# KLab/YAIK

Hardware: NVIDIA B200
Metric: encoded megapixels/sec (gradient+range stages) (higher is better)
Workload: dtype int32

## Files before the change

yaik_b200/csrc/yk_emit.cu:

```cuda
#include "yk_device.h"
#ifdef YK_EMULATE
#include <assert.h>
#endif

#ifndef YK_OWNER_THREADS
#define YK_OWNER_THREADS 256
#endif
static __device__ __forceinline__ int yk_owner_point(const YkSlotDev& S, int idx, const YkRun& run) {
    uint32_t word = __ldg(&S.touchMap[idx]);
    const int gy = idx / S.latW, gx = idx - gy * S.latW;
    if (S.hasAbove && gy == 0) word |= __ldg(&S.touchInTop[gx]);
    if (S.hasBelow && gy == S.latH - 1) word |= __ldg(&S.touchInBottom[gx]);
    if (word == 0u || (word & 0x80000000u)) return -1;
    const int rp = (__ffs((int)(word & 0x0FFFFFFFu)) - 1) >> 2;
    const unsigned nib = (word >> (4 * rp)) & 15u;
    const int pid = run.passId[rp];
    const YkGeomS g = yk_geom_s(pid);
    const int nSwzX = (S.w + (1 << g.lbw) - 1) >> g.lbw;
    const int LX = (4 * gx) >> g.shx, LY = (4 * gy) >> g.shy;
    const int tileRows = S.h >> g.shy;
    int best = INT_MAX, bestK = 0;
#pragma unroll
    for (int k = 0; k < 4; k++) {
        if ((nib >> k) & 1u) {
            const int ty = LY - (k >> 1);
            int pos;
            if (ty < 0) pos = k - 5;
            else if (ty >= tileRows) pos = INT_MAX - 1;
            else pos = yk_pos_s(g, nSwzX, LX - (k & 1), ty);
            if (pos < best) { best = pos; bestK = k; }
        }
    }
    if (best < 0 || best == INT_MAX - 1) return -1;
    atomicOr(&S.emitNib[pid][best >> 3], 1u << (4 * (best & 7) + bestK));
    return (pid << 24) | (int)((unsigned)(best >> 3) / YK_EMIT_THREADS);
}

static __device__ __forceinline__ void yk_rgb_add(const YkSlotDev& S, int key, unsigned bytes) {
    const unsigned grp = (unsigned)key & 0xFFFFFFu;
    atomicAdd(&S.rgbTot[key >> 24][grp], bytes);
    atomicAdd(&S.rgbSup[key >> 24][grp / YK_SUPER], bytes);
}
static __device__ __forceinline__ void yk_r2_add(const YkSlotDev& S, int grp, unsigned sum) {
    const unsigned long long v = (unsigned long long)(sum >> 16) << 32 | (sum & 0xFFFFu);
    atomicAdd(&S.r2Tot[grp], v);
    atomicAdd(&S.r2Sup[grp / YK_SUPER], v);
}

static __device__ __forceinline__ unsigned yk_r2_count(const YkSlotDev& S, int tx, int ty) {
    const uint32_t r0 = S.cellMask[(size_t)(2 * ty) * S.nbx + (tx >> 3)], r1 = S.cellMask[(size_t)(2 * ty + 1) * S.nbx + (tx >> 3)];
    const int s2 = 2 * (tx & 7);
    const unsigned chunks = 4u - (unsigned)__popc(((r0 >> s2) & 3u) | (((r1 >> s2) & 3u) << 2));
    return chunks ? chunks << 16 | 1u : 0u;
}

__global__ void __launch_bounds__(YK_OWNER_THREADS)
yk_k_owner(const YkSlotDev* __restrict__ slots, int slot0, int nPoints, int owners, YkRun run) {
    __shared__ int sKey[YK_NPASS + 1];
    __shared__ unsigned sSum[YK_NPASS + 1];
    if (threadIdx.x <= YK_NPASS) { sKey[threadIdx.x] = -1; sSum[threadIdx.x] = 0u; }
    __syncthreads();
    const YkSlotDev& S = slots[slot0 + blockIdx.y];
    const int idx = blockIdx.x * blockDim.x + threadIdx.x;
    const int lane = threadIdx.x & 31;
    const int key = owners && idx < nPoints ? yk_owner_point(S, idx, run) : -1;
    int r2Key = -1;
    unsigned r2 = 0u;
    if (run.doR2 && idx < nPoints) {
        const int gy = idx / S.latW, gx = idx - gy * S.latW, tx = gx >> 1, ty = gy >> 1;
        if (!((gx | gy) & 1) && tx < (S.w >> 3) && ty < (S.h >> 3)) {
            r2 = yk_r2_count(S, tx, ty);
            if (r2) r2Key = (int)((unsigned)(ty * (S.w >> 3) + tx) / YK_EMIT_THREADS);
        }
    }
    const unsigned rgbLanes = __ballot_sync(YK_FULL, key >= 0), r2Lanes = __ballot_sync(YK_FULL, r2Key >= 0);
    const int rgbTop = __reduce_max_sync(YK_FULL, key), r2Top = __reduce_max_sync(YK_FULL, r2Key);
    const bool rgbOne = __all_sync(YK_FULL, key < 0 || key == rgbTop), r2One = __all_sync(YK_FULL, r2Key < 0 || r2Key == r2Top);
    const unsigned r2Warp = __reduce_add_sync(YK_FULL, r2);
    const bool addRgb = key >= 0 && (!rgbOne || lane == __ffs((int)rgbLanes) - 1);
    const bool addR2 = r2Key >= 0 && (!r2One || lane == __ffs((int)r2Lanes) - 1);
    const unsigned rgbBytes = rgbOne ? 3u * (unsigned)__popc(rgbLanes) : 3u, r2Sum = r2One ? r2Warp : r2;
    if (addRgb) atomicMax(&sKey[key >> 24], key);
    if (addR2) atomicMax(&sKey[YK_NPASS], r2Key);
    __syncthreads();
    if (addRgb) {
        if (sKey[key >> 24] == key) atomicAdd(&sSum[key >> 24], rgbBytes);
        else yk_rgb_add(S, key, rgbBytes);
    }
    if (addR2) {
        if (sKey[YK_NPASS] == r2Key) atomicAdd(&sSum[YK_NPASS], r2Sum);
        else yk_r2_add(S, r2Key, r2Sum);
    }
    __syncthreads();
    if (threadIdx.x < YK_NPASS && sSum[threadIdx.x]) yk_rgb_add(S, sKey[threadIdx.x], sSum[threadIdx.x]);
    if (threadIdx.x == YK_NPASS && sSum[YK_NPASS]) yk_r2_add(S, sKey[YK_NPASS], sSum[YK_NPASS]);
}

static __device__ __forceinline__ void yk_emit_scan(unsigned c, unsigned d, unsigned pc, unsigned pd, unsigned& offC, unsigned& offD,
                                                    unsigned& totC, unsigned& totD) {
    constexpr int NW = YK_EMIT_THREADS / 32;
    __shared__ unsigned sC[NW], sD[NW], sPC[NW], sPD[NW], sTot[2];
    const int lane = threadIdx.x & 31, warp = threadIdx.x >> 5;
    unsigned ic = c, id = d;
#pragma unroll
    for (int k = 1; k < 32; k <<= 1) {
        const unsigned a0 = __shfl_up_sync(YK_FULL, ic, k), a1 = __shfl_up_sync(YK_FULL, id, k);
        if (lane >= k) { ic += a0; id += a1; }
    }
    pc = __reduce_add_sync(YK_FULL, pc); pd = __reduce_add_sync(YK_FULL, pd);
    if (lane == 31) { sC[warp] = ic; sD[warp] = id; }
    if (lane == 0) { sPC[warp] = pc; sPD[warp] = pd; }
    __syncthreads();
    if (warp == 0) {
        const unsigned a = lane < NW ? sC[lane] : 0u, b = lane < NW ? sD[lane] : 0u;
        const unsigned bc = __reduce_add_sync(YK_FULL, lane < NW ? sPC[lane] : 0u), bd = __reduce_add_sync(YK_FULL, lane < NW ? sPD[lane] : 0u);
        unsigned ia = a, ib = b;
#pragma unroll
        for (int k = 1; k < 32; k <<= 1) {
            const unsigned a0 = __shfl_up_sync(YK_FULL, ia, k), a1 = __shfl_up_sync(YK_FULL, ib, k);
            if (lane >= k) { ia += a0; ib += a1; }
        }
        if (lane < NW) { sC[lane] = bc + ia - a; sD[lane] = bd + ib - b; }
        if (lane == 31) { sTot[0] = ia; sTot[1] = ib; }
    }
    __syncthreads();
    offC = sC[warp] + ic - c; offD = sD[warp] + id - d;
    totC = sTot[0]; totD = sTot[1];
}

__global__ void __launch_bounds__(YK_EMIT_THREADS)
yk_k_emit(const YkSlotDev* __restrict__ slots, int slot0, YkRun run, int gradGroups, int r2Groups) {
    const YkSlotDev& S = slots[slot0 + blockIdx.y];
    const int tid = threadIdx.x;
    const int w = S.w, h = S.h;

    if ((int)blockIdx.x >= gradGroups) {
        const int grp = blockIdx.x - gradGroups, tilesW = w >> 3, nTiles = tilesW * (h >> 3);
        unsigned long long pre = tid < grp % YK_SUPER ? S.r2Tot[grp - grp % YK_SUPER + tid] : 0ull;
        for (int s = tid; s < grp / YK_SUPER; s += YK_EMIT_THREADS) pre += S.r2Sup[s];
        const int t = grp * YK_EMIT_THREADS + tid;
        const unsigned c = t < nTiles ? yk_r2_count(S, t % tilesW, t / tilesW) : 0u;
        const unsigned chunks = c >> 16;
        const unsigned tiles = chunks > 0;
        unsigned chunkOff, tileOff, totC, totT;
        yk_emit_scan(chunks, tiles, (unsigned)(pre >> 32), (unsigned)pre, chunkOff, tileOff, totC, totT);
#ifdef YK_EMULATE
        if (tid == 0) assert(((unsigned long long)totC << 32 | totT) == S.r2Tot[grp]);
#endif
        if (grp == r2Groups - 1 && tid == 0) { S.hdr[YK_HD_R2_CHUNKS] = (int)(chunkOff + totC); S.hdr[YK_HD_R2_TILES] = (int)(tileOff + totT); }
        if (chunks) {
#pragma unroll 1
            for (int p = 0; p < 3; p++) {
                const uint4* src = reinterpret_cast<const uint4*>(S.r2Raw[p] + (size_t)t * 64);
                uint4* dst = reinterpret_cast<uint4*>(S.r2Idx[p] + (size_t)chunkOff * 16);
                for (int k = 0; k < (int)chunks; k++) dst[k] = src[k];
                const uint32_t ty = S.r2RawType[p][t];
                uint8_t* td = S.r2Type[p] + (size_t)tileOff * 3;
                td[0] = (uint8_t)ty; td[1] = (uint8_t)(ty >> 8); td[2] = (uint8_t)(ty >> 16);
            }
        }
        return;
    }

    int rp = 0, grp = blockIdx.x, nWords = 0, nSwzX = 0, nGroups = 0;
    YkGeomS g = yk_geom_s(run.passId[0]);
    for (;;) {
        g = yk_geom_s(run.passId[rp]);
        nSwzX = (w + (1 << g.lbw) - 1) >> g.lbw;
        nWords = (nSwzX * ((h + (1 << g.lbh) - 1) >> g.lbh) * g.bits) >> 3;
        nGroups = (nWords + YK_EMIT_THREADS - 1) / YK_EMIT_THREADS;
        if (grp < nGroups) break;
        grp -= nGroups; rp++;
    }
    const int pid = run.passId[rp];
    unsigned pre = tid < grp % YK_SUPER ? S.rgbTot[pid][grp - grp % YK_SUPER + tid] : 0u;
    for (int s = tid; s < grp / YK_SUPER; s += YK_EMIT_THREADS) pre += S.rgbSup[pid][s];
    const int wi = grp * YK_EMIT_THREADS + tid;
    uint32_t word = wi < nWords ? __ldg(&S.emitNib[pid][wi]) : 0u;
    const unsigned cnt = 3u * (unsigned)__popc(word);
    unsigned off, tot, unused0, unused1;
    yk_emit_scan(cnt, 0u, pre, 0u, off, unused0, tot, unused1);
#ifdef YK_EMULATE
    if (tid == 0) assert(tot == S.rgbTot[pid][grp]);
#endif
    if (grp == nGroups - 1 && tid == 0) S.hdr[YK_HD_PASS0 + pid * YK_ST_STRIDE + YK_ST_RGBBYTES] = (int)(off + tot);
    if (word == 0u) return;
    const int lbits = g.bits == 16 ? 4 : (g.bits == 32 ? 5 : 6);
    const int pos0 = wi * 8, blk = pos0 >> lbits, within0 = pos0 & (g.bits - 1);
    const int tprShift = g.lbw - g.shx;
    const int bys = blk / nSwzX, bxs = blk - bys * nSwzX;
    uint8_t* out = S.rgb[pid];
    while (word) {
        const int b = __ffs((int)word) - 1;
        word &= word - 1u;
        const int within = within0 + (b >> 2), k = b & 3;
        const int gtx = (bxs << tprShift) + (within & ((1 << tprShift) - 1)), gty = (bys << (g.lbh - g.shy)) + (within >> tprShift);
        const int gx = ((gtx + (k & 1)) << g.shx) >> 2, gy = ((gty + (k >> 1)) << g.shy) >> 2;
        const uint8_t* sp = S.latRGB + ((size_t)gy * S.latW + gx) * 3;
        out[off] = sp[0]; out[off + 1] = sp[1]; out[off + 2] = sp[2];
        off += 3;
    }
}

void yk_launch_owner(const YkSlotDev* slotsDev, int slot0, int nSlots, int nPoints, bool owners, const YkRun& run, cudaStream_t st) {
    YK_LAUNCH(yk_k_owner, dim3((nPoints + YK_OWNER_THREADS - 1) / YK_OWNER_THREADS, nSlots), dim3(YK_OWNER_THREADS), 0, st, slotsDev, slot0, nPoints, owners ? 1 : 0, run);
}
void yk_launch_emit(const YkSlotDev* slotsDev, int slot0, int nSlots, int gradGroups, int r2Groups, const YkRun& run, cudaStream_t st) {
    YK_LAUNCH(yk_k_emit, dim3(gradGroups + r2Groups, nSlots), dim3(YK_EMIT_THREADS), 0, st, slotsDev, slot0, run, gradGroups, r2Groups);
}

__global__ void yk_k_flag_set(unsigned* a, unsigned* b, unsigned value) {
    __threadfence_system();
    if (a) yk_stv(a, value);
    if (b) yk_stv(b, value);
}
__global__ void yk_k_flag_wait(const unsigned* a, const unsigned* b, unsigned value) {
    while (a && (int)(yk_ldv(a) - value) < 0) yk_spin();
    while (b && (int)(yk_ldv(b) - value) < 0) yk_spin();
    __threadfence_system();
}
void yk_launch_flag_set(unsigned* a, unsigned* b, unsigned value, cudaStream_t st) { YK_LAUNCH(yk_k_flag_set, dim3(1), dim3(1), 0, st, a, b, value); }
void yk_launch_flag_wait(const unsigned* a, const unsigned* b, unsigned value, cudaStream_t st) { YK_LAUNCH(yk_k_flag_wait, dim3(1), dim3(1), 0, st, a, b, value); }

int yk_preload_emit() {
#ifndef YK_EMULATE
    cudaFuncAttributes fa;
    { const cudaError_t e = cudaFuncGetAttributes(&fa, yk_k_owner); if (e != cudaSuccess) return (int)e; }
    { const cudaError_t e = cudaFuncGetAttributes(&fa, yk_k_emit); if (e != cudaSuccess) return (int)e; }
    { const cudaError_t e = cudaFuncGetAttributes(&fa, yk_k_flag_set); if (e != cudaSuccess) return (int)e; }
    { const cudaError_t e = cudaFuncGetAttributes(&fa, yk_k_flag_wait); if (e != cudaSuccess) return (int)e; }
#endif
    return 0;
}
```

Baseline: 96080.

## Compact emit work into shared lists for coalesced block-wide copies

The emit kernel now builds a shared-memory list of corner indices, or chunk indices for the r2 path, after the scan. The whole block then copies the RGB triples and uint4 chunks cooperatively with coalesced output writes, instead of each thread serially walking its own bits. The owner kernel hoists its loads, packs pass ids into registers, and issues the emitNib atomicOr before the first barrier. This removes per-thread serialization and divergent strided writes, at the cost of extra barriers, shared memory and some redundant bit walking per round.

```diff
diff --git a/yaik_b200/csrc/yk_emit.cu b/yaik_b200/csrc/yk_emit.cu
--- a/yaik_b200/csrc/yk_emit.cu
+++ b/yaik_b200/csrc/yk_emit.cu
@@ -6,19 +6,22 @@
 #ifndef YK_OWNER_THREADS
 #define YK_OWNER_THREADS 256
 #endif
-static __device__ __forceinline__ int yk_owner_point(const YkSlotDev& S, int idx, const YkRun& run) {
-    uint32_t word = __ldg(&S.touchMap[idx]);
-    const int gy = idx / S.latW, gx = idx - gy * S.latW;
-    if (S.hasAbove && gy == 0) word |= __ldg(&S.touchInTop[gx]);
-    if (S.hasBelow && gy == S.latH - 1) word |= __ldg(&S.touchInBottom[gx]);
-    if (word == 0u || (word & 0x80000000u)) return -1;
+static __device__ __forceinline__ unsigned yk_pass_ids(const YkRun& run) {
+    unsigned v = 0u;
+#pragma unroll
+    for (int i = 0; i < YK_NPASS; i++) v |= ((unsigned)run.passId[i] & 15u) << (4 * i);
+    return v;
+}
+static __device__ __forceinline__ int yk_pass_at(unsigned ids, int rp) { return (int)(ids >> (4 * rp)) & 15; }
+
+static __device__ __forceinline__ int yk_owner_point(int w, int h, uint32_t word, int gx, int gy, unsigned passIds, int& posK) {
     const int rp = (__ffs((int)(word & 0x0FFFFFFFu)) - 1) >> 2;
     const unsigned nib = (word >> (4 * rp)) & 15u;
-    const int pid = run.passId[rp];
+    const int pid = yk_pass_at(passIds, rp);
     const YkGeomS g = yk_geom_s(pid);
-    const int nSwzX = (S.w + (1 << g.lbw) - 1) >> g.lbw;
+    const int nSwzX = (w + (1 << g.lbw) - 1) >> g.lbw;
     const int LX = (4 * gx) >> g.shx, LY = (4 * gy) >> g.shy;
-    const int tileRows = S.h >> g.shy;
+    const int tileRows = h >> g.shy;
     int best = INT_MAX, bestK = 0;
 #pragma unroll
     for (int k = 0; k < 4; k++) {
@@ -32,26 +35,29 @@
         }
     }
     if (best < 0 || best == INT_MAX - 1) return -1;
-    atomicOr(&S.emitNib[pid][best >> 3], 1u << (4 * (best & 7) + bestK));
+    posK = best << 2 | bestK;
     return (pid << 24) | (int)((unsigned)(best >> 3) / YK_EMIT_THREADS);
 }
 
-static __device__ __forceinline__ void yk_rgb_add(const YkSlotDev& S, int key, unsigned bytes) {
+static __device__ __forceinline__ void yk_rgb_add(uint32_t* tot, uint32_t* sup, int key, unsigned bytes) {
     const unsigned grp = (unsigned)key & 0xFFFFFFu;
-    atomicAdd(&S.rgbTot[key >> 24][grp], bytes);
-    atomicAdd(&S.rgbSup[key >> 24][grp / YK_SUPER], bytes);
-}
-static __device__ __forceinline__ void yk_r2_add(const YkSlotDev& S, int grp, unsigned sum) {
+    atomicAdd(&tot[grp], bytes);
+    atomicAdd(&sup[grp / YK_SUPER], bytes);
+}
+static __device__ __forceinline__ void yk_r2_add(unsigned long long* tot, unsigned long long* sup, int grp, unsigned sum) {
     const unsigned long long v = (unsigned long long)(sum >> 16) << 32 | (sum & 0xFFFFu);
-    atomicAdd(&S.r2Tot[grp], v);
-    atomicAdd(&S.r2Sup[grp / YK_SUPER], v);
-}
-
-static __device__ __forceinline__ unsigned yk_r2_count(const YkSlotDev& S, int tx, int ty) {
-    const uint32_t r0 = S.cellMask[(size_t)(2 * ty) * S.nbx + (tx >> 3)], r1 = S.cellMask[(size_t)(2 * ty + 1) * S.nbx + (tx >> 3)];
+    atomicAdd(&tot[grp], v);
+    atomicAdd(&sup[grp / YK_SUPER], v);
+}
+
+static __device__ __forceinline__ unsigned yk_r2_rule(uint32_t r0, uint32_t r1, int tx) {
     const int s2 = 2 * (tx & 7);
     const unsigned chunks = 4u - (unsigned)__popc(((r0 >> s2) & 3u) | (((r1 >> s2) & 3u) << 2));
     return chunks ? chunks << 16 | 1u : 0u;
+}
+static __device__ __forceinline__ unsigned yk_r2_count(const YkSlotDev& S, int tx, int ty) {
+    const uint16_t* cm = S.cellMask + (size_t)(2 * ty) * S.nbx + (tx >> 3);
+    return yk_r2_rule(cm[0], cm[S.nbx], tx);
 }
 
 __global__ void __launch_bounds__(YK_OWNER_THREADS)
@@ -59,20 +65,40 @@
     __shared__ int sKey[YK_NPASS + 1];
     __shared__ unsigned sSum[YK_NPASS + 1];
     if (threadIdx.x <= YK_NPASS) { sKey[threadIdx.x] = -1; sSum[threadIdx.x] = 0u; }
-    __syncthreads();
     const YkSlotDev& S = slots[slot0 + blockIdx.y];
     const int idx = blockIdx.x * blockDim.x + threadIdx.x;
     const int lane = threadIdx.x & 31;
-    const int key = owners && idx < nPoints ? yk_owner_point(S, idx, run) : -1;
+    const int w = S.w, h = S.h, latW = S.latW, gy = idx / latW, gx = idx - gy * latW;
+    const bool r2Point = run.doR2 && idx < nPoints && !((gx | gy) & 1) && (gx >> 1) < (w >> 3) && (gy >> 1) < (h >> 3);
+    uint32_t word = 0u, m0 = 0u, m1 = 0u;
+    if (owners && idx < nPoints) {
+        word = __ldg(&S.touchMap[idx]);
+        if (S.hasAbove && gy == 0) word |= __ldg(&S.touchInTop[gx]);
+        if (S.hasBelow && gy == S.latH - 1) word |= __ldg(&S.touchInBottom[gx]);
+    }
+    if (r2Point) {
+        const int nbx = S.nbx;
+        const uint16_t* cm = S.cellMask + (size_t)gy * nbx + (gx >> 4);
+        m0 = __ldg(cm); m1 = __ldg(cm + nbx);
+    }
+    uint32_t* const finTot = threadIdx.x < YK_NPASS ? S.rgbTot[threadIdx.x] : nullptr;
+    uint32_t* const finSup = threadIdx.x < YK_NPASS ? S.rgbSup[threadIdx.x] : nullptr;
+    unsigned long long* const r2Tot = run.doR2 ? S.r2Tot : nullptr;
+    unsigned long long* const r2Sup = run.doR2 ? S.r2Sup : nullptr;
+
+    int key = -1, posK = 0;
+    if (word != 0u && !(word & 0x80000000u))
+        key = yk_owner_point(w, h, word, gx, gy, yk_pass_ids(run), posK);
+    uint32_t *nib = nullptr, *tot = nullptr, *sup = nullptr;
+    if (key >= 0) { nib = S.emitNib[key >> 24]; tot = S.rgbTot[key >> 24]; sup = S.rgbSup[key >> 24]; }
     int r2Key = -1;
     unsigned r2 = 0u;
-    if (run.doR2 && idx < nPoints) {
-        const int gy = idx / S.latW, gx = idx - gy * S.latW, tx = gx >> 1, ty = gy >> 1;
-        if (!((gx | gy) & 1) && tx < (S.w >> 3) && ty < (S.h >> 3)) {
-            r2 = yk_r2_count(S, tx, ty);
-            if (r2) r2Key = (int)((unsigned)(ty * (S.w >> 3) + tx) / YK_EMIT_THREADS);
-        }
-    }
+    if (r2Point) {
+        r2 = yk_r2_rule(m0, m1, gx >> 1);
+        if (r2) r2Key = (int)((unsigned)((gy >> 1) * (w >> 3) + (gx >> 1)) / YK_EMIT_THREADS);
+    }
+    if (key >= 0) atomicOr(&nib[posK >> 5], 1u << (posK & 31));
+    __syncthreads();
     const unsigned rgbLanes = __ballot_sync(YK_FULL, key >= 0), r2Lanes = __ballot_sync(YK_FULL, r2Key >= 0);
     const int rgbTop = __reduce_max_sync(YK_FULL, key), r2Top = __reduce_max_sync(YK_FULL, r2Key);
     const bool rgbOne = __all_sync(YK_FULL, key < 0 || key == rgbTop), r2One = __all_sync(YK_FULL, r2Key < 0 || r2Key == r2Top);
@@ -85,21 +111,21 @@
     __syncthreads();
     if (addRgb) {
         if (sKey[key >> 24] == key) atomicAdd(&sSum[key >> 24], rgbBytes);
-        else yk_rgb_add(S, key, rgbBytes);
+        else yk_rgb_add(tot, sup, key, rgbBytes);
     }
     if (addR2) {
         if (sKey[YK_NPASS] == r2Key) atomicAdd(&sSum[YK_NPASS], r2Sum);
-        else yk_r2_add(S, r2Key, r2Sum);
-    }
-    __syncthreads();
-    if (threadIdx.x < YK_NPASS && sSum[threadIdx.x]) yk_rgb_add(S, sKey[threadIdx.x], sSum[threadIdx.x]);
-    if (threadIdx.x == YK_NPASS && sSum[YK_NPASS]) yk_r2_add(S, sKey[YK_NPASS], sSum[YK_NPASS]);
+        else yk_r2_add(r2Tot, r2Sup, r2Key, r2Sum);
+    }
+    __syncthreads();
+    if (threadIdx.x < YK_NPASS && sSum[threadIdx.x]) yk_rgb_add(finTot, finSup, sKey[threadIdx.x], sSum[threadIdx.x]);
+    if (threadIdx.x == YK_NPASS && sSum[YK_NPASS]) yk_r2_add(r2Tot, r2Sup, sKey[YK_NPASS], sSum[YK_NPASS]);
 }
 
 static __device__ __forceinline__ void yk_emit_scan(unsigned c, unsigned d, unsigned pc, unsigned pd, unsigned& offC, unsigned& offD,
-                                                    unsigned& totC, unsigned& totD) {
+                                                    unsigned& baseC, unsigned& baseD, unsigned& totC, unsigned& totD) {
     constexpr int NW = YK_EMIT_THREADS / 32;
-    __shared__ unsigned sC[NW], sD[NW], sPC[NW], sPD[NW], sTot[2];
+    __shared__ unsigned sC[NW], sD[NW], sPC[NW], sPD[NW], sTot[4];
     const int lane = threadIdx.x & 31, warp = threadIdx.x >> 5;
     unsigned ic = c, id = d;
 #pragma unroll
@@ -120,85 +146,139 @@
             const unsigned a0 = __shfl_up_sync(YK_FULL, ia, k), a1 = __shfl_up_sync(YK_FULL, ib, k);
             if (lane >= k) { ia += a0; ib += a1; }
         }
-        if (lane < NW) { sC[lane] = bc + ia - a; sD[lane] = bd + ib - b; }
-        if (lane == 31) { sTot[0] = ia; sTot[1] = ib; }
+        if (lane < NW) { sC[lane] = ia - a; sD[lane] = ib - b; }
+        if (lane == 31) { sTot[0] = ia; sTot[1] = ib; sTot[2] = bc; sTot[3] = bd; }
     }
     __syncthreads();
     offC = sC[warp] + ic - c; offD = sD[warp] + id - d;
-    totC = sTot[0]; totD = sTot[1];
-}
-
-__global__ void __launch_bounds__(YK_EMIT_THREADS)
+    totC = sTot[0]; totD = sTot[1]; baseC = sTot[2]; baseD = sTot[3];
+}
+
+#ifndef YK_EMIT_LIST
+#define YK_EMIT_LIST (4 * YK_EMIT_THREADS)
+#endif
+static_assert(YK_EMIT_LIST % YK_EMIT_THREADS == 0, "YK_EMIT_LIST: whole corners per thread");
+
+__global__ void __launch_bounds__(YK_EMIT_THREADS, 2048 / YK_EMIT_THREADS)
 yk_k_emit(const YkSlotDev* __restrict__ slots, int slot0, YkRun run, int gradGroups, int r2Groups) {
+    constexpr int T = YK_EMIT_THREADS;
+    __shared__ uint32_t sList[YK_EMIT_LIST > 2 * T ? YK_EMIT_LIST : 2 * T];
     const YkSlotDev& S = slots[slot0 + blockIdx.y];
     const int tid = threadIdx.x;
     const int w = S.w, h = S.h;
 
     if ((int)blockIdx.x >= gradGroups) {
         const int grp = blockIdx.x - gradGroups, tilesW = w >> 3, nTiles = tilesW * (h >> 3);
+        const int t0 = grp * T, t = t0 + tid;
         unsigned long long pre = tid < grp % YK_SUPER ? S.r2Tot[grp - grp % YK_SUPER + tid] : 0ull;
-        for (int s = tid; s < grp / YK_SUPER; s += YK_EMIT_THREADS) pre += S.r2Sup[s];
-        const int t = grp * YK_EMIT_THREADS + tid;
+        for (int s = tid; s < grp / YK_SUPER; s += T) pre += S.r2Sup[s];
         const unsigned c = t < nTiles ? yk_r2_count(S, t % tilesW, t / tilesW) : 0u;
+        uint32_t ty0 = 0u, ty1 = 0u, ty2 = 0u;
+        if (t < nTiles) { ty0 = __ldg(&S.r2RawType[0][t]); ty1 = __ldg(&S.r2RawType[1][t]); ty2 = __ldg(&S.r2RawType[2][t]); }
+        __shared__ const uint8_t* sRaw[3];
+        __shared__ uint8_t *sIdx[3], *sType[3];
+        if (tid < 3) { sRaw[tid] = S.r2Raw[tid]; sIdx[tid] = S.r2Idx[tid]; sType[tid] = S.r2Type[tid]; }
         const unsigned chunks = c >> 16;
-        const unsigned tiles = chunks > 0;
-        unsigned chunkOff, tileOff, totC, totT;
-        yk_emit_scan(chunks, tiles, (unsigned)(pre >> 32), (unsigned)pre, chunkOff, tileOff, totC, totT);
+        unsigned chunkOff, tileOff, chunkBase, tileBase, totC, totT;
+        yk_emit_scan(chunks, chunks > 0, (unsigned)(pre >> 32), (unsigned)pre, chunkOff, tileOff, chunkBase, tileBase, totC, totT);
 #ifdef YK_EMULATE
         if (tid == 0) assert(((unsigned long long)totC << 32 | totT) == S.r2Tot[grp]);
 #endif
-        if (grp == r2Groups - 1 && tid == 0) { S.hdr[YK_HD_R2_CHUNKS] = (int)(chunkOff + totC); S.hdr[YK_HD_R2_TILES] = (int)(tileOff + totT); }
+        if (grp == r2Groups - 1 && tid == 0) { S.hdr[YK_HD_R2_CHUNKS] = (int)(chunkBase + totC); S.hdr[YK_HD_R2_TILES] = (int)(tileBase + totT); }
+        uint16_t* const sChunk = reinterpret_cast<uint16_t*>(sList);
+        for (unsigned k = 0; k < chunks; k++) sChunk[chunkOff + k] = (uint16_t)(tid << 2 | k);
         if (chunks) {
-#pragma unroll 1
-            for (int p = 0; p < 3; p++) {
-                const uint4* src = reinterpret_cast<const uint4*>(S.r2Raw[p] + (size_t)t * 64);
-                uint4* dst = reinterpret_cast<uint4*>(S.r2Idx[p] + (size_t)chunkOff * 16);
-                for (int k = 0; k < (int)chunks; k++) dst[k] = src[k];
-                const uint32_t ty = S.r2RawType[p][t];
-                uint8_t* td = S.r2Type[p] + (size_t)tileOff * 3;
-                td[0] = (uint8_t)ty; td[1] = (uint8_t)(ty >> 8); td[2] = (uint8_t)(ty >> 16);
+            const size_t td = (size_t)(tileBase + tileOff) * 3;
+            uint8_t *const d0 = sType[0] + td, *const d1 = sType[1] + td, *const d2 = sType[2] + td;
+            d0[0] = (uint8_t)ty0; d0[1] = (uint8_t)(ty0 >> 8); d0[2] = (uint8_t)(ty0 >> 16);
+            d1[0] = (uint8_t)ty1; d1[1] = (uint8_t)(ty1 >> 8); d1[2] = (uint8_t)(ty1 >> 16);
+            d2[0] = (uint8_t)ty2; d2[1] = (uint8_t)(ty2 >> 8); d2[2] = (uint8_t)(ty2 >> 16);
+        }
+        __syncthreads();
+        const unsigned nItems = 3u * totC;
+        for (unsigned i0 = tid; i0 < nItems; i0 += 4 * T) {
+            uint4 v[4];
+#pragma unroll
+            for (int u = 0; u < 4; u++) {
+                const unsigned i = i0 + u * T;
+                if (i < nItems) {
+                    const unsigned p = i >= totC ? (i >= 2 * totC ? 2u : 1u) : 0u, e = sChunk[i - p * totC];
+                    v[u] = __ldg(reinterpret_cast<const uint4*>(sRaw[p] + (size_t)(t0 + (e >> 2)) * 64) + (e & 3));
+                }
+            }
+#pragma unroll
+            for (int u = 0; u < 4; u++) {
+                const unsigned i = i0 + u * T;
+                if (i < nItems) {
+                    const unsigned p = i >= totC ? (i >= 2 * totC ? 2u : 1u) : 0u;
+                    reinterpret_cast<uint4*>(sIdx[p])[chunkBase + i - p * totC] = v[u];
+                }
             }
         }
         return;
     }
 
+    const unsigned passIds = yk_pass_ids(run);
     int rp = 0, grp = blockIdx.x, nWords = 0, nSwzX = 0, nGroups = 0;
-    YkGeomS g = yk_geom_s(run.passId[0]);
+    YkGeomS g;
     for (;;) {
-        g = yk_geom_s(run.passId[rp]);
+        g = yk_geom_s(yk_pass_at(passIds, rp));
         nSwzX = (w + (1 << g.lbw) - 1) >> g.lbw;
         nWords = (nSwzX * ((h + (1 << g.lbh) - 1) >> g.lbh) * g.bits) >> 3;
-        nGroups = (nWords + YK_EMIT_THREADS - 1) / YK_EMIT_THREADS;
+        nGroups = (nWords + T - 1) / T;
         if (grp < nGroups) break;
         grp -= nGroups; rp++;
     }
-    const int pid = run.passId[rp];
+    const int pid = yk_pass_at(passIds, rp);
     unsigned pre = tid < grp % YK_SUPER ? S.rgbTot[pid][grp - grp % YK_SUPER + tid] : 0u;
-    for (int s = tid; s < grp / YK_SUPER; s += YK_EMIT_THREADS) pre += S.rgbSup[pid][s];
-    const int wi = grp * YK_EMIT_THREADS + tid;
-    uint32_t word = wi < nWords ? __ldg(&S.emitNib[pid][wi]) : 0u;
-    const unsigned cnt = 3u * (unsigned)__popc(word);
-    unsigned off, tot, unused0, unused1;
-    yk_emit_scan(cnt, 0u, pre, 0u, off, unused0, tot, unused1);
+    for (int s = tid; s < grp / YK_SUPER; s += T) pre += S.rgbSup[pid][s];
+    const int wi = grp * T + tid;
+    const uint32_t word = wi < nWords ? __ldg(&S.emitNib[pid][wi]) : 0u;
+    const uint8_t* const lat = S.latRGB;
+    const int latW = S.latW;
+    const unsigned mine = (unsigned)__popc(word);
+    unsigned first, base, nCorners, unused0, unused1, unused2;
+    yk_emit_scan(mine, 0u, pre, 0u, first, unused0, base, unused1, nCorners, unused2);
 #ifdef YK_EMULATE
-    if (tid == 0) assert(tot == S.rgbTot[pid][grp]);
-#endif
-    if (grp == nGroups - 1 && tid == 0) S.hdr[YK_HD_PASS0 + pid * YK_ST_STRIDE + YK_ST_RGBBYTES] = (int)(off + tot);
-    if (word == 0u) return;
+    if (tid == 0) assert(3u * nCorners == S.rgbTot[pid][grp]);
+#endif
+    if (grp == nGroups - 1 && tid == 0) S.hdr[YK_HD_PASS0 + pid * YK_ST_STRIDE + YK_ST_RGBBYTES] = (int)(base + 3u * nCorners);
+    uint8_t* const out = S.rgb[pid] + base;
     const int lbits = g.bits == 16 ? 4 : (g.bits == 32 ? 5 : 6);
     const int pos0 = wi * 8, blk = pos0 >> lbits, within0 = pos0 & (g.bits - 1);
     const int tprShift = g.lbw - g.shx;
     const int bys = blk / nSwzX, bxs = blk - bys * nSwzX;
-    uint8_t* out = S.rgb[pid];
-    while (word) {
-        const int b = __ffs((int)word) - 1;
-        word &= word - 1u;
-        const int within = within0 + (b >> 2), k = b & 3;
-        const int gtx = (bxs << tprShift) + (within & ((1 << tprShift) - 1)), gty = (bys << (g.lbh - g.shy)) + (within >> tprShift);
-        const int gx = ((gtx + (k & 1)) << g.shx) >> 2, gy = ((gty + (k >> 1)) << g.shy) >> 2;
-        const uint8_t* sp = S.latRGB + ((size_t)gy * S.latW + gx) * 3;
-        out[off] = sp[0]; out[off + 1] = sp[1]; out[off + 2] = sp[2];
-        off += 3;
+    for (unsigned r0 = 0; r0 < nCorners; r0 += YK_EMIT_LIST) {
+        if (first < r0 + YK_EMIT_LIST && first + mine > r0) {
+            uint32_t rest = word;
+            for (unsigned i = first; rest && i < r0 + YK_EMIT_LIST; i++) {
+                const int b = __ffs((int)rest) - 1;
+                rest &= rest - 1u;
+                if (i < r0) continue;
+                const int within = within0 + (b >> 2), k = b & 3;
+                const int gtx = (bxs << tprShift) + (within & ((1 << tprShift) - 1)), gty = (bys << (g.lbh - g.shy)) + (within >> tprShift);
+                const int gx = ((gtx + (k & 1)) << g.shx) >> 2, gy = ((gty + (k >> 1)) << g.shy) >> 2;
+                sList[i - r0] = (uint32_t)(gy * latW + gx);
+            }
+        }
+        __syncthreads();
+        const unsigned n = min(nCorners - r0, (unsigned)YK_EMIT_LIST);
+        constexpr int K = YK_EMIT_LIST / T;
+#pragma unroll
+        for (int u0 = 0; u0 < K; u0 += 2) {
+            uint8_t v[2][3];
+#pragma unroll
+            for (int u = 0; u < 2; u++) {
+                const unsigned j = tid + (u0 + u) * T;
+                if (u0 + u < K && j < n) { const uint8_t* sp = lat + (size_t)sList[j] * 3; v[u][0] = __ldg(sp); v[u][1] = __ldg(sp + 1); v[u][2] = __ldg(sp + 2); }
+            }
+#pragma unroll
+            for (int u = 0; u < 2; u++) {
+                const unsigned j = tid + (u0 + u) * T;
+                if (u0 + u < K && j < n) { uint8_t* dp = out + (size_t)(r0 + j) * 3; dp[0] = v[u][0]; dp[1] = v[u][1]; dp[2] = v[u][2]; }
+            }
+        }
+        if (r0 + YK_EMIT_LIST < nCorners) __syncthreads();
     }
 }
 
```

After: 100,800, median of 6. 4.9% higher.
